# apache/paimon

Measured on AMD Instinct MI355X. Metric: merged rows/sec, higher is better.
Workload: dtype int64; 1 GPU; merge-on-read: 8 sorted runs x 10000000 rows, int64 PK + 8 int32, parquet NONE, Deduplicate, drop-delete (BASELINE.json configs[1]); n_runs=8, rows_per_run=10000000, compression=NONE, seed=42, parallelism=bucket-parallel dp1, no collectives

## Files before the change

### include/paimon_hip.h

```cpp
#ifndef PAIMON_HIP_H
#define PAIMON_HIP_H

#include <stdint.h>

#ifdef __cplusplus
extern "C" {
#endif

typedef struct pmh_session_t pmh_session_t;
typedef struct pmh_plan_t pmh_plan_t;

enum pmh_dtype {
    PMH_DT_INT8 = 1,
    PMH_DT_INT16 = 2,
    PMH_DT_INT32 = 3,
    PMH_DT_INT64 = 4,
    PMH_DT_FLOAT32 = 5,
    PMH_DT_FLOAT64 = 6,
    PMH_DT_STRING = 7,
    PMH_DT_BOOL = 8,
};

enum pmh_logical {
    PMH_LT_NONE = 0,
// ... 92 lines not shown
                              int scale, int64_t n_values, int out_esize,
                              int mode, int64_t src_shift, void *out,
                              int64_t out_cap);

int64_t pmh_debug_bits(const void *stream, int64_t len, int64_t n_values,
                       int bit_order, int format, int out_esize, int mode,
                       int64_t src_shift, int64_t out_shift, void *out,
                       int64_t out_cap);

int64_t pmh_debug_orc_timestamp(const void *data, int64_t data_len,
                                const void *secondary, int64_t secondary_len,
                                int64_t n_values, int unit, int mode,
                                void *out, int64_t out_cap);

int64_t pmh_debug_parse_dv(const char *path, int64_t offset, int64_t length,
                           int64_t *out, int64_t cap);

int pmh_debug_lookup_probe(int n_levels, const int64_t *const *level_keys,
                           const int64_t *level_rows, const int64_t *queries,
                           int64_t n_queries, int32_t *out_level,
                           int64_t *out_row);

int pmh_debug_changelog_decide(int64_t n_groups, const int32_t *nlive,
                               const int32_t *n_top,
                               const uint8_t *merged_is_add, int pending,
                               int32_t *out_n, int8_t *out_kinds,
                               uint8_t *out_after_is_merged,
                               uint8_t *out_pending);

int pmh_debug_partition(int k, const void *const *keys, const int64_t *lens,
                        int key_width, int64_t tile_rows, int mode,
                        int32_t *cuts_out);

int pmh_debug_json_i64(const char *text, int64_t *out);

int pmh_debug_interval_partition(int n, const int64_t *min_keys,
                                 const int64_t *max_keys,
                                 int32_t *out_section, int32_t *out_run);

#ifdef __cplusplus
}
#endif
#endif
```

### paimon_amd/csrc/kernels.h

```cpp
#pragma once

#include <hip/hip_runtime.h>

#include <cstdint>

#include "bits_core.h"
#include "orc_decimal_core.h"
#include "orc_timestamp_core.h"
#include "stream_core.h"

namespace pmh {

constexpr int PMH_MAX_RUNS = 32;
constexpr int PMH_ROW_BITS = 27;
constexpr uint32_t PMH_ROW_MASK = ((uint32_t)1 << PMH_ROW_BITS) - 1;
constexpr int PMH_TILE_THREADS = 512;
constexpr int64_t PMH_TILE_ROWS = 3584;
constexpr int PMH_COARSE_G = 16;
constexpr int64_t PMH_DEAD = INT64_MIN;
constexpr int PMH_TILE_MAX = PMH_TILE_ROWS + PMH_MAX_RUNS;
constexpr int PMH_TILE_ITER =
    (PMH_TILE_MAX + PMH_TILE_THREADS - 1) / PMH_TILE_THREADS;

struct DevPage {
// ... 121 lines not shown

hipError_t pmh_launch_scan_tiles(const int32_t *tile_counts, int64_t n_tiles,
                                 int64_t *tile_offsets, int64_t *total_out,
                                 hipStream_t stream);

hipError_t pmh_launch_merge_emit(const DevCol *keys, const DevCol *seqs,
                                 const DevCol *kinds, const int64_t *lens,
                                 int k, const int32_t *cuts,
                                 int64_t tile_base, int64_t tile_limit,
                                 int64_t n_tiles,
                                 int64_t tile_rows, int flags,
                                 const uint64_t *tombs,
                                 const DevCol *cols, const uint8_t *col_dtype,
                                 const uint8_t *col_nullable, int n_cols,
                                 int key_col, int seq_col, int kind_col,
                                 const int16_t *useq_cols, int n_useq,
                                 uint64_t *status, uint64_t *ticket,
                                 int64_t *total_out, uint32_t *dense_winners,
                                 void *const *out_ptrs,
                                 uint8_t *const *out_valid,
                                 uint32_t *err_flag, hipStream_t stream);

hipError_t pmh_launch_emit_dense(const DevCol *cols,
                                 const uint8_t *col_dtype,
                                 const uint8_t *col_nullable, int n_cols,
                                 int key_col, int seq_col, int kind_col,
                                 const uint32_t *winners,
                                 int64_t t0, int64_t t1,
                                 const uint64_t *status,
                                 void *const *out_ptrs,
                                 uint8_t *const *out_valid,
                                 hipStream_t stream);

hipError_t pmh_launch_emit(const DevCol *cols, const uint8_t *col_dtype,
                           const uint8_t *col_nullable, int n_cols, int k,
                           int n_desc, int contiguous,
                           const uint32_t *winners,
                           const int32_t *tile_counts,
                           const int64_t *tile_offsets, int64_t n_tiles,
                           int64_t tile_rows, const int64_t *total_out,
                           void *const *out_ptrs, uint8_t *const *out_valid,
                           hipStream_t stream);

hipError_t pmh_launch_rle_decode(const RleChunk *chunks, int64_t n_chunks,
                                 int32_t *out, hipStream_t stream);

hipError_t pmh_launch_level_scatter(const RleChunk *chunks, int64_t n_chunks,
                                    hipStream_t stream);

hipError_t pmh_launch_emit_pu(const DevCol *cols, const uint8_t *col_dtype,
                              const uint8_t *col_nullable, int n_cols, int k,
                              int seq_col, int kind_col, int flags,
                              const uint32_t *members,
                              const uint16_t *group_start,
                              const int64_t *tile_offsets, int64_t n_tiles,
                              int64_t tile_rows, const int64_t *total_out,
                              uint64_t *const *run_masks,
                              void *const *out_ptrs,
                              uint8_t *const *out_valid, hipStream_t stream);

hipError_t pmh_launch_pack_valid(const DevCol *cols, int n_cols, int64_t rows,
                                 uint64_t *mask, hipStream_t stream);

hipError_t pmh_launch_composite(const DevCol *keys, int nk, uint64_t shifts,
                                uint64_t bits, int64_t rows, int64_t *ckey,
                                hipStream_t stream);

enum {
    PMH_AGG_LAST_NON_NULL = 0,
// ... 39 lines not shown
```

### paimon_amd/csrc/kernels.hip

```cpp

#include <hip/hip_runtime.h>

#include <cstdint>
#include <cstdlib>
#include <type_traits>

#include "changelog_core.h"
#include "kernels.h"
#include "lookup_core.h"
#include "partition_core.h"
#include "zstd_core.h"

#define DEV __device__ __forceinline__

namespace pmh {


template <typename T>
DEV T col_load(const DevCol &c, int64_t row) {
    if (c.n_pages == 1)
        return *reinterpret_cast<const T *>(c.addr0 + (uint64_t)row * sizeof(T));
    int lo = 0, hi = c.n_pages - 1;
    while (lo < hi) {
        int mid = (lo + hi + 1) >> 1;
        if (c.pages[mid].start_row <= row) lo = mid;
        else hi = mid - 1;
    }
    const DevPage &pg = c.pages[lo];
    return *reinterpret_cast<const T *>(pg.addr + (uint64_t)(row - pg.start_row) * sizeof(T));
}

DEV uint64_t ukey(int64_t k) { return (uint64_t)k ^ 0x8000000000000000ull; }

DEV int64_t key_at(uint64_t addr, int64_t idx, int es) {
    return es == 8 ? *reinterpret_cast<const int64_t *>(addr + idx * 8)
                   : (int64_t)*reinterpret_cast<const int32_t *>(addr +
                                                                 idx * 4);
}


// ... 1991 lines not shown
            } else {
                wa[x] = wa[0];
            }
        }
        uint32_t packed[R];
#pragma unroll
        for (int x = 0; x < R; x++) packed[x] = gload<uint32_t>(wa[x]);
        int dl[R];
        uint32_t row[R];
#pragma unroll
        for (int x = 0; x < R; x++) {
            dl[x] = (int)(packed[x] >> PMH_ROW_BITS) * n_cols;
            row[x] = packed[x] & PMH_ROW_MASK;
        }
        auto lists = [&](auto full) {
            constexpr bool FULL = decltype(full)::value;
            const uint32_t utid = (uint32_t)tid;
            emit_list<int32_t, int8_t, G4, R, FULL>(
                s_addr, s_valid, s_out, s_ov, 0, e1, dl, row, base, utid, nr);
            emit_list<int32_t, int16_t, G4, R, FULL>(
                s_addr, s_valid, s_out, s_ov, e1, e2, dl, row, base, utid, nr);
            emit_list<int32_t, int32_t, G4, R, FULL>(
                s_addr, s_valid, s_out, s_ov, e2, e4, dl, row, base, utid, nr);
            emit_list<int64_t, int64_t, G8, R, FULL>(
                s_addr, s_valid, s_out, s_ov, e4, e8, dl, row, base, utid, nr);
        };
        if (base + (int64_t)EMIT_THREADS * R <= slice_hi)
            lists(std::true_type{});
        else
            lists(std::false_type{});
    }
}

__global__ void k_composite(const DevCol *keys, int nk, uint64_t shifts,
                            uint64_t bits, int64_t rows, int64_t *ckey) {
    const int64_t stride = (int64_t)gridDim.x * blockDim.x;
    for (int64_t i = (int64_t)blockIdx.x * blockDim.x + threadIdx.x; i < rows;
         i += stride) {
        uint64_t u = 0;
        for (int j = 0; j < nk; j++) {
            const DevCol &dc = keys[j];
            int64_t v = dc.esize == 8 ? col_load<int64_t>(dc, i)
                                      : (int64_t)col_load<int32_t>(dc, i);
            const int w = (int)((bits >> (8 * j)) & 0xff);
            const int sh = (int)((shifts >> (8 * j)) & 0xff);
            uint64_t b = ((uint64_t)v + (1ull << (w - 1))) &
                         (w >= 64 ? ~0ull : ((1ull << w) - 1));
            u |= b << sh;
        }
        ckey[i] = (int64_t)(u ^ 0x8000000000000000ull);
    }
}

__global__ void k_pack_valid(const DevCol *cols, int n_cols, int64_t rows,
                             uint64_t *mask) {
    const int64_t stride = (int64_t)gridDim.x * blockDim.x;
    for (int64_t i = (int64_t)blockIdx.x * blockDim.x + threadIdx.x; i < rows;
         i += stride) {
        uint64_t m = 0;
        for (int c = 0; c < n_cols; c++) {
            const DevCol &dc = cols[c];
            uint64_t v =
                dc.valid0 ? (uint64_t)((const uint8_t *)dc.valid0)[i] : 1u;
            m |= (v & 1) << c;
        }
        mask[i] = m;
// ... 2294 lines not shown
    };
    if (fr)
        launch(k_merge_emit<true>);
    else
        launch(k_merge_emit<false>);
    return hipGetLastError();
}

hipError_t pmh_launch_emit_dense(const DevCol *cols,
                                 const uint8_t *col_dtype,
                                 const uint8_t *col_nullable, int n_cols,
                                 int key_col, int seq_col, int kind_col,
                                 const uint32_t *winners,
                                 int64_t t0, int64_t t1,
                                 const uint64_t *status,
                                 void *const *out_ptrs,
                                 uint8_t *const *out_valid,
                                 hipStream_t stream) {
    hipLaunchKernelGGL(k_emit_dense, dim3(emit_grid()), dim3(256), 0, stream, cols,
                       col_dtype, col_nullable, n_cols, key_col, seq_col,
                       kind_col, winners, t0, t1, status, out_ptrs,
                       out_valid);
    return hipGetLastError();
}

hipError_t pmh_launch_scan_tiles(const int32_t *tile_counts, int64_t n_tiles,
                                 int64_t *tile_offsets, int64_t *total_out,
                                 hipStream_t stream) {
    hipLaunchKernelGGL(k_scan_tiles, dim3(1), dim3(PMH_TILE_THREADS), 0,
                       stream, tile_counts, n_tiles, tile_offsets, total_out);
    return hipGetLastError();
}

hipError_t pmh_launch_emit(const DevCol *cols, const uint8_t *col_dtype,
                           const uint8_t *col_nullable, int n_cols, int k,
                           int n_desc, int contiguous,
                           const uint32_t *winners,
                           const int32_t *tile_counts,
                           const int64_t *tile_offsets, int64_t n_tiles,
                           int64_t tile_rows, const int64_t *total_out,
                           void *const *out_ptrs, uint8_t *const *out_valid,
                           hipStream_t stream) {
    auto env_int = [](const char *name, int dflt) {
        const char *e = getenv(name);
        return e ? atoi(e) : dflt;
    };
    const int r_rows = env_int("PMH_EMIT_R", 4);
    const int g_cols = env_int("PMH_EMIT_G", 8);
    int n_emit = env_int("PMH_EMIT_COLS", n_cols);
    if (n_emit < 0 || n_emit > n_cols) n_emit = n_cols;
    const int grid = emit_grid();
    const int64_t lds = emit_contig_lds(n_desc, n_cols);
    const bool contig = contiguous && n_desc >= 1 && n_cols <= 256 &&
                        lds <= EMIT_LDS_MAX &&
                        env_int("PMH_EMIT_LEGACY", 0) == 0;
    if (contig) {
        auto launch = [&](auto kern) {
            hipLaunchKernelGGL(kern, dim3(grid), dim3(EMIT_THREADS), (size_t)lds,
                               stream, cols, col_dtype, col_nullable, n_cols,
                               n_emit, n_desc, winners, tile_offsets, n_tiles,
                               tile_rows, total_out, out_ptrs, out_valid);
        };
        if (r_rows == 2) {
            if (g_cols == 2) launch(k_emit_contig<2, 2, 1>);
            else if (g_cols == 4) launch(k_emit_contig<2, 4, 2>);
            else launch(k_emit_contig<2, 8, 4>);
        } else {
            if (g_cols == 2) launch(k_emit_contig<4, 2, 1>);
            else if (g_cols == 4) launch(k_emit_contig<4, 4, 2>);
            else if (g_cols == 16) launch(k_emit_contig<4, 16, 8>);
            else launch(k_emit_contig<4, 8, 4>);
        }
        return hipGetLastError();
    }
    auto launch = [&](auto kern) {
        hipLaunchKernelGGL(kern, dim3(grid), dim3(256), 0, stream, cols,
                           col_dtype, col_nullable, n_cols, n_emit, k,
                           winners, tile_counts, tile_offsets, n_tiles,
                           tile_rows, total_out, out_ptrs, out_valid);
    };
    if (r_rows == 6)
        launch(k_emit<6>);
    else if (r_rows == 8)
        launch(k_emit<8>);
    else
        launch(k_emit<4>);
    return hipGetLastError();
}
// ... 210 lines not shown
```

### paimon_amd/csrc/plan.cpp

```cpp

#include <hip/hip_runtime.h>

#include <algorithm>
#include <chrono>
#include <cstring>
#include <fstream>
#include <memory>
#include <queue>
#include <string>
#include <unordered_map>
#include <vector>

#include "../../include/paimon_hip.h"
#include "changelog_core.h"
#include "codec.h"
#include "zstd_core.h"
#include <map>
#include "common.h"
#include "json.h"
#include "kernels.h"
#include "lookup_core.h"
#include "orc_meta.h"
#include "parquet_meta.h"
#include "parquet_write.h"
// ... 3536 lines not shown
        const char *dwhat = "decode";
        hipError_t de = launch_section_decode(p, sec, st, &dwhat);
        if (de != hipSuccess) return fail(dwhat, de);
    }
    if (p->composite_key) {
        for (int r = 0; r < k; r++) {
            if (sec.runs[r].length <= 0) continue;
            hipError_t ce = pmh_launch_composite(
                sec.all_cols + (size_t)r * n_cols, p->n_key_cols,
                p->key_shifts, p->key_bits, sec.runs[r].length, sec.ckeys[r],
                st);
            if (ce != hipSuccess) return fail("composite", ce);
        }
    }
    if (sec.row_masks_dev) {
        for (int r = 0; r < k; r++) {
            if (sec.runs[r].length <= 0) continue;
            hipError_t pe = pmh_launch_pack_valid(
                sec.all_cols + (size_t)r * n_cols, n_cols,
                sec.runs[r].length, sec.row_masks[r], st);
            if (pe != hipSuccess) return fail("pack_valid", pe);
        }
    }
    (void)hipEventRecord(ev[1], st);
    if (p->filters_dev && k == 1 && !sec.hier && sec.runs[0].tomb &&
        sec.runs[0].length > 0) {
        hipError_t fe = pmh_launch_filter(
            sec.all_cols, n_cols, p->filters_dev, (int)p->filters.size(),
            sec.runs[0].length, sec.runs[0].tomb, st);
        if (fe != hipSuccess) return fail("filter", fe);
    }
    int64_t n_tiles_eff = sec.n_tiles;
    int64_t rows_eff = sec.total_rows;
    if (sec.hier) {
        const int nb = (int)sec.blo.size();
        k = nb;
        const int bflags = p->first_row ? 8 : 0;
        for (int b = 0; b < nb; b++) {
            int lo = sec.blo[b];
            int kb = sec.bhi[b] - lo;
            int64_t btiles = sec.bntiles[b];
            hipError_t hb = pmh_launch_partition(
                sec.rkeys + lo, sec.rlens + lo, kb, PMH_TILE_ROWS,
                btiles + 1, sec.brows[b], sec.cuts, st);
            if (hb != hipSuccess) return fail("hier partition", hb);
            hb = pmh_launch_merge_tiles(
                sec.rkeys + lo, sec.rseqs + lo, sec.rkinds + lo,
                sec.rlens + lo, kb, sec.cuts, btiles, PMH_TILE_ROWS, bflags,
                sec.rtombs ? sec.rtombs + lo : nullptr, sec.winners,
                sec.tile_counts, sec.group_start, sec.err_dev, nullptr, 0,
                nullptr, nullptr, nullptr, nullptr, st);
            if (hb != hipSuccess) return fail("hier merge", hb);
            hb = pmh_launch_scan_tiles(sec.tile_counts, btiles,
                                       sec.tile_offsets, sec.lens_dev + b,
                                       st);
            if (hb != hipSuccess) return fail("hier scan", hb);
            hb = pmh_launch_emit(sec.rall + (size_t)lo * n_cols,
                                 p->hier_dtype_dev, p->col_nullable_dev,
                                 n_cols, kb, kb, sec.cols_contig,
                                 sec.winners, sec.tile_counts,
                                 sec.tile_offsets, btiles, PMH_TILE_ROWS,
                                 sec.lens_dev + b, sec.bout_ptrs[b],
                                 sec.bout_valid[b], st);
            if (hb != hipSuccess) return fail("hier emit", hb);
        }
        std::vector<int64_t> vl(nb);
        if (hipMemcpy(vl.data(), sec.lens_dev, nb * 8,
                      hipMemcpyDeviceToHost) != hipSuccess)
            return fail("hier lens D2H", hipErrorUnknown);
        rows_eff = 0;
        for (int b = 0; b < nb; b++) rows_eff += vl[b];
        n_tiles_eff = (rows_eff + PMH_TILE_ROWS - 1) / PMH_TILE_ROWS;
        if (n_tiles_eff == 0) n_tiles_eff = 1;
    }
    hipError_t e = pmh_launch_partition(sec.key_cols, sec.lens_dev, k,
                                        PMH_TILE_ROWS, n_tiles_eff + 1,
                                        rows_eff, sec.cuts, st);
    if (e != hipSuccess) return fail("partition", e);
    (void)hipEventRecord(ev[2], st);
    int flags = (p->drop_delete ? 1 : 0) | (p->ignore_delete ? 2 : 0) |
                (p->pu ? 4 : 0) | (p->first_row ? 8 : 0) |
                (p->rrod ? 16 : 0) | (p->seqg ? 32 : 0) |
                (p->agg_retract ? 64 : 0);
    if (const char *ab = getenv("PMH_ABLATE"))
        flags |= (atoi(ab) & 0xf) << 8;
    if (const char *ab = getenv("PMH_FABL"))
        flags |= (atoi(ab) & 0x3) << 12;
    if (const char *fs = getenv("PMH_FSTAGE"))
        flags |= (atoi(fs) & 1) << 14;
    if (p->fused) {
        e = hipMemsetAsync(sec.status, 0, n_tiles_eff * 8, st);
        if (e != hipSuccess) return fail("status memset", e);
// ... 86 lines not shown
                               sec.run_levels, p->max_level, sec.cl_entries,
                               sec.cl_counts, sec.probe_words, sec.probe_off,
                               st);
    if (e != hipSuccess) return fail("merge_tiles", e);
    (void)hipEventRecord(ev[3], st);
    e = pmh_launch_scan_tiles(sec.tile_counts, n_tiles_eff, sec.tile_offsets,
                              sec.total_dev, st);
    if (e != hipSuccess) return fail("scan_tiles", e);
    (void)hipEventRecord(ev[4], st);
    if (p->agg) {
        e = pmh_launch_emit_agg(
            sec.all_cols, p->col_dtype_dev, p->col_nullable_dev,
            p->col_agg_dev, n_cols, k, p->n_key_cols, p->n_key_cols + 1,
            flags, sec.winners, sec.group_start, sec.tile_offsets,
            n_tiles_eff, PMH_TILE_ROWS, sec.total_dev, sec.row_masks_dev,
            p->out_ptrs_dev, p->out_valid_dev, st);
    } else if (p->pu && p->seqg) {
        e = pmh_launch_emit_pu_sg(
            sec.all_cols, p->col_dtype_dev, p->col_nullable_dev, n_cols, k,
            p->n_key_cols, p->n_key_cols + 1, flags, p->col_group_dev,
            p->sg_fields_dev, p->sg_nseq_dev, p->n_seq_groups, sec.winners,
            sec.group_start, sec.tile_offsets, n_tiles_eff, PMH_TILE_ROWS,
            sec.total_dev, sec.row_masks_dev, p->out_ptrs_dev,
            p->out_valid_dev, st);
    } else if (p->pu) {
        e = pmh_launch_emit_pu(
            sec.all_cols, p->col_dtype_dev, p->col_nullable_dev, n_cols, k,
            p->n_key_cols, p->n_key_cols + 1, flags, sec.winners,
            sec.group_start, sec.tile_offsets, n_tiles_eff, PMH_TILE_ROWS,
            sec.total_dev, sec.row_masks_dev, p->out_ptrs_dev,
            p->out_valid_dev, st);
    } else {
        e = pmh_launch_emit(sec.all_cols, p->col_dtype_dev,
                            p->col_nullable_dev, n_cols, k,
                            sec.hier ? k : k + sec.n_lookup,
                            sec.hier || sec.cols_contig, sec.winners,
                            sec.tile_counts, sec.tile_offsets, n_tiles_eff,
                            PMH_TILE_ROWS, sec.total_dev, p->out_ptrs_dev,
                            p->out_valid_dev, st);
    }
    if (e != hipSuccess) return fail("emit", e);
    if (p->cl_fold) {
        e = pmh_launch_cl_finalize_out(
            sec.all_cols, p->col_dtype_dev, p->col_nullable_dev, n_cols,
            p->n_key_cols + 2, k, sec.cl_entries, sec.cl_rows, sec.cl_counts,
            sec.tile_offsets, n_tiles_eff, PMH_TILE_ROWS, p->out_ptrs_dev,
            p->out_valid_dev, st);
        if (e != hipSuccess) return fail("cl_finalize_out", e);
        e = pmh_launch_scan_tiles(sec.cl_counts, n_tiles_eff, sec.cl_offsets,
                                  sec.cl_total_dev, st);
        if (e != hipSuccess) return fail("cl_scan", e);
        e = pmh_launch_cl_emit_out(
            sec.all_cols, p->col_dtype_dev, p->col_nullable_dev, n_cols, k,
            p->n_key_cols + 1, sec.cl_rows, sec.cl_counts, sec.cl_offsets,
            sec.tile_offsets, n_tiles_eff, PMH_TILE_ROWS, p->out_ptrs_dev,
            p->out_valid_dev, p->out_ptrs2_dev, p->out_valid2_dev, st);
        if (e != hipSuccess) return fail("cl_emit_out", e);
    } else if (p->changelog) {
        e = pmh_launch_cl_finalize(sec.all_cols, p->col_dtype_dev, n_cols,
                                   p->n_key_cols + 2, k, sec.cl_entries,
                                   sec.cl_rows, sec.cl_counts, n_tiles_eff,
                                   PMH_TILE_ROWS, st);
        if (e != hipSuccess) return fail("cl_finalize", e);
        e = pmh_launch_scan_tiles(sec.cl_counts, n_tiles_eff, sec.cl_offsets,
                                  sec.cl_total_dev, st);
        if (e != hipSuccess) return fail("cl_scan", e);
        e = pmh_launch_cl_emit(sec.all_cols, p->col_dtype_dev,
                               p->col_nullable_dev, n_cols,
                               p->n_key_cols + 1, sec.cl_rows, sec.cl_counts,
// ... 986 lines not shown
    }
    return 0;
}

int pmh_debug_changelog_decide(int64_t n_groups, const int32_t *nlive,
                               const int32_t *n_top,
                               const uint8_t *merged_is_add, int pending,
                               int32_t *out_n, int8_t *out_kinds,
                               uint8_t *out_after_is_merged,
                               uint8_t *out_pending) {
    if (n_groups < 0 ||
        (n_groups > 0 && (!nlive || !n_top || !merged_is_add || !out_n ||
                          !out_kinds))) {
        set_error("pmh_debug_changelog_decide: bad arguments");
        return -1;
    }
    for (int64_t g = 0; g < n_groups; g++) {
        if (nlive[g] < 1 || n_top[g] < 0 || n_top[g] > nlive[g]) {
            set_error("pmh_debug_changelog_decide: group %lld is malformed "
                      "(nlive >= 1, 0 <= n_top <= nlive)", (long long)g);
            return -1;
        }
        const ClcDecision d = clc_decide(nlive[g], n_top[g],
                                         merged_is_add[g] != 0, pending != 0);
        out_n[g] = d.n;
        out_kinds[2 * g] = (int8_t)(d.n >= 1 ? d.kind0 : -1);
        out_kinds[2 * g + 1] = (int8_t)(d.n == 2 ? d.kind1 : -1);
        if (out_after_is_merged) out_after_is_merged[g] = d.after_is_merged;
        if (out_pending) out_pending[g] = d.pending;
    }
    return 0;
}

int pmh_debug_partition(int k, const void *const *keys, const int64_t *lens,
                        int key_width, int64_t tile_rows, int mode,
                        int32_t *cuts_out) {
    if (k < 1 || k > PMH_MAX_RUNS || !keys || !lens || !cuts_out ||
        (key_width != 4 && key_width != 8) || tile_rows < 1 ||
        (mode != 0 && mode != 1)) {
        set_error("pmh_debug_partition: bad arguments (1..%d runs, key_width "
                  "4|8, tile_rows >= 1, mode 0|1)", PMH_MAX_RUNS);
        return -1;
    }
    int64_t total = 0;
    for (int r = 0; r < k; r++) {
        if (lens[r] < 0 || lens[r] >= ((int64_t)1 << PMH_ROW_BITS) ||
            (lens[r] > 0 && !keys[r])) {
            set_error("pmh_debug_partition: run %d is malformed", r);
            return -1;
        }
        total += lens[r];
    }
    const int64_t n_bounds = (total + tile_rows - 1) / tile_rows + 1;
    if (mode == 0) {
        const int64_t G = k <= 8 ? (n_bounds > PMH_COARSE_G + 1 ? PMH_COARSE_G
                                                                 : 1)
                                 : (n_bounds > 1 ? n_bounds - 1 : 1);
        static_assert(PPC_MAX_RUNS == PMH_MAX_RUNS, "widest instantiation");
        ppc_host_partition(k, keys, lens, key_width, tile_rows, n_bounds,
                           total, G, cuts_out);
        return 0;
    }
    constexpr int GUARD = 64;
    const size_t n_cuts = (size_t)n_bounds * k;
    std::vector<void *> bufs;
    auto dalloc = [&](size_t n) -> void * {
// ... 102 lines not shown
```

### paimon_amd/reader.py

```python

import ctypes
import json
import os

import numpy as np

_HERE = os.path.dirname(os.path.abspath(__file__))
LIB_PATH = os.path.join(_HERE, "libpaimon_hip.so")

_DT_NP = {1: np.int8, 2: np.int16, 3: np.int32, 4: np.int64,
          5: np.float32, 6: np.float64,
          7: np.int32,
          8: np.bool_}

(LT_NONE, LT_DATE, LT_TIME_MILLIS, LT_TIMESTAMP_MILLIS, LT_TIMESTAMP_MICROS,
 LT_TIMESTAMP_LTZ_MILLIS, LT_TIMESTAMP_LTZ_MICROS) = range(7)


class _Col(ctypes.Structure):
    _fields_ = [("name", ctypes.c_char_p), ("dtype", ctypes.c_int32),
                ("data", ctypes.c_void_p), ("valid", ctypes.c_void_p),
                ("dict_data", ctypes.c_void_p),
                ("dict_offsets", ctypes.POINTER(ctypes.c_int32)),
                ("dict_len", ctypes.c_int32),
# ... 399 lines not shown
    return out_level, out_row


PARTITION_HOST = 0
PARTITION_DEVICE = 1


def debug_partition(runs, tile_rows, mode=PARTITION_HOST):
    lib = load_lib()
    dt = np.dtype(runs[0].dtype)
    if dt not in (np.dtype(np.int64), np.dtype(np.int32)):
        raise ValueError("keys must be int64 or int32")
    ks = [np.ascontiguousarray(a, dtype=dt) for a in runs]
    k = len(ks)
    total = sum(len(a) for a in ks)
    n_bounds = (total + tile_rows - 1) // tile_rows + 1
    ptrs = (ctypes.c_void_p * k)(
        *[a.ctypes.data if len(a) else None for a in ks])
    lens = (ctypes.c_int64 * k)(*[len(a) for a in ks])
    cuts = np.empty((n_bounds, k), dtype=np.int32)
    lib.pmh_debug_partition.restype = ctypes.c_int
    lib.pmh_debug_partition.argtypes = [
        ctypes.c_int, ctypes.POINTER(ctypes.c_void_p),
        ctypes.POINTER(ctypes.c_int64), ctypes.c_int, ctypes.c_int64,
        ctypes.c_int, ctypes.POINTER(ctypes.c_int32)]
    rc = lib.pmh_debug_partition(
        k, ptrs, lens, dt.itemsize, tile_rows, mode,
        cuts.ctypes.data_as(ctypes.POINTER(ctypes.c_int32)))
    if rc != 0:
        raise RuntimeError(last_error())
    return cuts


class Session:
    def __init__(self, device=0):
        self.lib = load_lib()
        self.h = self.lib.pmh_open_session(device)
        if not self.h:
            raise RuntimeError(f"pmh_open_session: {last_error()}")
        self.device = device

    def close(self):
        if self.h:
            self.lib.pmh_close_session(self.h)
            self.h = None

    def __enter__(self):
        return self

    def __exit__(self, *a):
        self.close()


class MergeReadPlan:

    def __init__(self, session: Session, files, key_cols, value_cols,
                 merge_engine="deduplicate", drop_delete=True,
                 ignore_delete=False, output="host", aggregations=None,
                 remove_record_on_delete=False, sequence_groups=None,
                 ignore_retract=None, sequence_fields=None,
                 changelog_producer=None, changelog_row_dedup=False,
                 max_level=None, sort_engine="loser-tree", filters=None,
                 lookup_files=None):
        self.lib = session.lib
        desc = {
            "key_cols": key_cols,
# ... 134 lines not shown
```

Measured before the change: 20.87 billion rows/s.

## Add streamed LDS-staged emit kernel that gathers tile source rows then permutes winners

Adds a new emit path for contiguous, non-nullable inputs. Each tile's source rows are read coalesced from the sorted runs and grouped by column width into LDS. Winners are then gathered from LDS via slot indices computed from the tile cuts. The loads for the next column group or next tile are issued before the current permute, overlapping global reads with LDS work. This replaces scattered random global gathers with sequential loads, at the cost of reading loser rows too, added LDS pressure and barriers, and a more complex persistent-grid schedule.

```diff
diff --git a/include/paimon_hip.h b/include/paimon_hip.h
--- a/include/paimon_hip.h
+++ b/include/paimon_hip.h
@@ -148,6 +148,8 @@
                         int key_width, int64_t tile_rows, int mode,
                         int32_t *cuts_out);
 
+int pmh_debug_last_emit_kernel(void);
+
 int pmh_debug_json_i64(const char *text, int64_t *out);
 
 int pmh_debug_interval_partition(int n, const int64_t *min_keys,
diff --git a/paimon_amd/csrc/emit_stream_core.h b/paimon_amd/csrc/emit_stream_core.h
--- /dev/null
+++ b/paimon_amd/csrc/emit_stream_core.h
@@ -0,0 +1,101 @@
+#ifndef PMH_EMIT_STREAM_CORE_H
+#define PMH_EMIT_STREAM_CORE_H
+
+#include <stdint.h>
+
+#if defined(__HIPCC__)
+#define ESC_HD __host__ __device__ __forceinline__
+#else
+#define ESC_HD inline
+#endif
+#if defined(__clang__)
+#define ESC_UNROLL _Pragma("unroll")
+#else
+#define ESC_UNROLL
+#endif
+
+template <int KM>
+struct EscTile {
+    int32_t a[KM];
+    int32_t len[KM];
+    int32_t segoff[KM];
+    int32_t mtotal;
+    int32_t mreal;
+};
+
+template <int KM>
+ESC_HD void esc_tile_setup(const int32_t *c0, const int32_t *c1,
+                           const int64_t *lens, int k, EscTile<KM> &t) {
+    int32_t so = 0, mr = 0;
+    ESC_UNROLL
+    for (int r = 0; r < KM; r++) {
+        const int rr = r < k ? r : 0;
+        const int32_t ar = c0[rr], br = c1[rr];
+        const int32_t ln = (int32_t)lens[rr];
+        t.a[r] = ar;
+        t.len[r] = r < k ? (br - ar) + (br < ln ? 1 : 0) : 0;
+        t.segoff[r] = so;
+        so += t.len[r];
+        mr += r < k ? br - ar : 0;
+    }
+    t.mtotal = so;
+    t.mreal = mr;
+}
+
+template <int KM>
+ESC_HD void esc_slot_source(const EscTile<KM> &t, int k, int32_t e, int *run,
+                            uint32_t *row) {
+    int rn = 0;
+    int32_t rowd = 0;
+    ESC_UNROLL
+    for (int r = 0; r < KM; r++) {
+        const bool in = r < k && e >= t.segoff[r];
+        rn = in ? r : rn;
+        rowd = in ? t.a[r] - t.segoff[r] : rowd;
+    }
+    *run = rn;
+    *row = (uint32_t)(e + rowd);
+}
+
+template <int KM>
+ESC_HD int32_t esc_winner_slot(const EscTile<KM> &t, uint32_t run,
+                               uint32_t row) {
+    int32_t off = 0;
+    ESC_UNROLL
+    for (int r = 0; r < KM; r++)
+        off = run == (uint32_t)r ? t.segoff[r] - t.a[r] : off;
+    return (int32_t)row + off;
+}
+
+ESC_HD int esc_stored_width(int cls) { return cls == 8 ? 8 : 4; }
+
+ESC_HD int64_t esc_col_bytes(int cls, int has_valid, int tile_max) {
+    return (int64_t)tile_max * (esc_stored_width(cls) + (has_valid ? 1 : 0));
+}
+
+ESC_HD int esc_plan_groups(const uint8_t *cls, const uint8_t *valid, int n,
+                           int tile_max, int64_t budget, int max4, int max8,
+                           uint16_t *bound) {
+    int g = 0;
+    bound[0] = 0;
+    int i = 0;
+    while (i < n) {
+        const int c = cls[i];
+        const int cap = esc_stored_width(c) == 8 ? max8 : max4;
+        int64_t used = 0;
+        int j = i;
+        while (j < n && cls[j] == c && j - i < cap) {
+            const int64_t b =
+                esc_col_bytes(c, valid ? valid[j] : 0, tile_max);
+            if (used + b > budget) break;
+            used += b;
+            j++;
+        }
+        if (j == i) return -1;
+        bound[++g] = (uint16_t)j;
+        i = j;
+    }
+    return g;
+}
+
+#endif
diff --git a/paimon_amd/csrc/emit_stream_hostcheck.cpp b/paimon_amd/csrc/emit_stream_hostcheck.cpp
--- /dev/null
+++ b/paimon_amd/csrc/emit_stream_hostcheck.cpp
@@ -0,0 +1,237 @@
+#include "emit_stream_core.h"
+
+#include <cstdio>
+#include <cstdlib>
+#include <random>
+#include <vector>
+
+static int failures = 0;
+
+#define CHECK(cond)                                                        \
+    do {                                                                   \
+        if (!(cond)) {                                                     \
+            fprintf(stderr, "%s:%d: CHECK failed: %s\n", __FILE__,         \
+                    __LINE__, #cond);                                      \
+            failures++;                                                    \
+        }                                                                  \
+    } while (0)
+
+static const int MAX_RUNS = 32;
+static const int64_t TILE_ROWS = 3584;
+static const int TILE_MAX = (int)TILE_ROWS + MAX_RUNS;
+
+static std::vector<int32_t> gen_cuts(const std::vector<int64_t> &lens,
+                                     std::mt19937_64 &rng, int skew) {
+    const int k = (int)lens.size();
+    int64_t total = 0;
+    for (int64_t l : lens) total += l;
+    const int64_t n_tiles = total ? (total + TILE_ROWS - 1) / TILE_ROWS : 1;
+    std::vector<int32_t> cuts((size_t)(n_tiles + 1) * k, 0);
+    std::vector<int64_t> at(k, 0);
+    for (int64_t b = 1; b <= n_tiles; b++) {
+        int64_t want = b * TILE_ROWS < total ? TILE_ROWS
+                                             : total - (b - 1) * TILE_ROWS;
+        while (want > 0) {
+            int r = (int)(rng() % k);
+            if (skew && (rng() % (unsigned)(skew + 1)))
+                r = (int)(rng() % (unsigned)((k + 1) / 2));
+            if (at[r] >= lens[r]) {
+                r = -1;
+                for (int q = 0; q < k; q++)
+                    if (at[q] < lens[q]) r = q;
+                if (r < 0) break;
+            }
+            int64_t take = 1 + (int64_t)(rng() % 97);
+            if (take > want) take = want;
+            if (take > lens[r] - at[r]) take = lens[r] - at[r];
+            at[r] += take;
+            want -= take;
+        }
+        for (int r = 0; r < k; r++) cuts[(size_t)b * k + r] = (int32_t)at[r];
+    }
+    return cuts;
+}
+
+template <int KM>
+static void check_tiles(const std::vector<int64_t> &lens,
+                        const std::vector<int32_t> &cuts) {
+    const int k = (int)lens.size();
+    const int64_t n_tiles = (int64_t)cuts.size() / k - 1;
+    CHECK(k <= KM);
+    std::vector<int64_t> hl(lens);
+    for (int64_t t = 0; t < n_tiles; t++) {
+        std::vector<int32_t> c0(cuts.begin() + t * k,
+                                cuts.begin() + (t + 1) * k);
+        std::vector<int32_t> c1(cuts.begin() + (t + 1) * k,
+                                cuts.begin() + (t + 2) * k);
+        EscTile<KM> ts;
+        esc_tile_setup<KM>(c0.data(), c1.data(), hl.data(), k, ts);
+        const int32_t M = ts.mtotal;
+        CHECK(M >= 0 && M <= TILE_MAX);
+        int64_t real = 0, ext = 0;
+        for (int r = 0; r < k; r++) {
+            real += c1[r] - c0[r];
+            ext += c1[r] < lens[r] ? 1 : 0;
+        }
+        CHECK(ts.mreal == real);
+        CHECK(M == real + ext);
+        CHECK(real <= TILE_ROWS);
+        for (int32_t e = 0; e < M; e++) {
+            int run = -1;
+            uint32_t row = 0;
+            esc_slot_source<KM>(ts, k, e, &run, &row);
+            CHECK(run >= 0 && run < k);
+            if (run < 0 || run >= k) continue;
+            CHECK((int64_t)row >= c0[run] && (int64_t)row <= c1[run]);
+            CHECK((int64_t)row < lens[run]);
+            CHECK(esc_winner_slot<KM>(ts, (uint32_t)run, row) == e);
+        }
+        std::vector<uint8_t> hit((size_t)M, 0);
+        int64_t named = 0;
+        for (int r = 0; r < k; r++) {
+            for (int64_t row = c0[r]; row <= c1[r] && row < lens[r]; row++) {
+                const int32_t s =
+                    esc_winner_slot<KM>(ts, (uint32_t)r, (uint32_t)row);
+                CHECK(s >= 0 && s < M);
+                if (s < 0 || s >= M) continue;
+                CHECK(!hit[(size_t)s]);
+                hit[(size_t)s] = 1;
+                named++;
+            }
+        }
+        CHECK(named == M);
+    }
+}
+
+static void check_runs(const std::vector<int64_t> &lens,
+                       const std::vector<int32_t> &cuts) {
+    const int k = (int)lens.size();
+    if (k <= 4) check_tiles<4>(lens, cuts);
+    if (k <= 8) check_tiles<8>(lens, cuts);
+    if (k <= 16) check_tiles<16>(lens, cuts);
+    check_tiles<32>(lens, cuts);
+}
+
+static void tiles() {
+    std::mt19937_64 rng(20240611);
+    const int ks[] = {1, 2, 3, 8, 32};
+    for (int k : ks) {
+        for (int rep = 0; rep < 6; rep++) {
+            std::vector<int64_t> lens(k);
+            for (int r = 0; r < k; r++)
+                lens[r] = (int64_t)(rng() % (rep < 2 ? 300 : 9000));
+            if (rep == 3) lens[0] = 1;
+            if (rep == 4) lens[k - 1] = 0;
+            if (rep == 5 && k > 1) lens[1] = 20000;
+            check_runs(lens, gen_cuts(lens, rng, rep >= 3 ? 3 : 0));
+        }
+    }
+    {
+        const int64_t totals[] = {TILE_ROWS, TILE_ROWS + 1, 2 * TILE_ROWS, 100};
+        for (int64_t tot : totals) {
+            std::vector<int64_t> one{tot};
+            check_runs(one, gen_cuts(one, rng, 0));
+            std::vector<int64_t> three{1, tot / 2, tot - tot / 2 - 1};
+            check_runs(three, gen_cuts(three, rng, 2));
+        }
+    }
+    {
+        const int k = MAX_RUNS;
+        const int64_t per = TILE_ROWS / k;
+        std::vector<int64_t> lens(k, 2 * per);
+        std::vector<int32_t> cuts((size_t)3 * k, 0);
+        for (int r = 0; r < k; r++) {
+            cuts[(size_t)k + r] = (int32_t)per;
+            cuts[(size_t)2 * k + r] = (int32_t)(2 * per);
+        }
+        check_tiles<32>(lens, cuts);
+        EscTile<32> ts;
+        esc_tile_setup<32>(cuts.data(), cuts.data() + k, lens.data(), k, ts);
+        CHECK(ts.mtotal == TILE_MAX);
+        esc_tile_setup<32>(cuts.data() + k, cuts.data() + 2 * k, lens.data(),
+                           k, ts);
+        CHECK(ts.mtotal == TILE_ROWS);
+    }
+    {
+        std::vector<int64_t> lens{10, 5000};
+        std::vector<int32_t> cuts{0, 0, 10, 3574, 10, 5000};
+        check_runs(lens, cuts);
+    }
+}
+
+static void check_plan(const std::vector<uint8_t> &cls,
+                       const std::vector<uint8_t> *valid, int64_t budget,
+                       int max4, int max8) {
+    const int n = (int)cls.size();
+    std::vector<uint16_t> bound((size_t)n + 1, 0xffff);
+    const int g = esc_plan_groups(cls.data(), valid ? valid->data() : nullptr,
+                                  n, TILE_MAX, budget, max4, max8,
+                                  bound.data());
+    bool fits = true;
+    for (int i = 0; i < n; i++)
+        fits = fits &&
+               esc_col_bytes(cls[i], valid ? (*valid)[i] : 0, TILE_MAX) <=
+                   budget;
+    if (!fits) {
+        CHECK(g == -1);
+        return;
+    }
+    CHECK(g >= (n ? 1 : 0) && g <= n);
+    if (g < 0) return;
+    CHECK(bound[0] == 0 && bound[(size_t)g] == n);
+    for (int i = 0; i < g; i++) {
+        const int lo = bound[(size_t)i], hi = bound[(size_t)i + 1];
+        CHECK(lo < hi && hi <= n);
+        if (!(lo < hi && hi <= n)) return;
+        int64_t bytes = 0;
+        for (int c = lo; c < hi; c++) {
+            CHECK(cls[c] == cls[lo]);
+            bytes += esc_col_bytes(cls[c], valid ? (*valid)[c] : 0, TILE_MAX);
+        }
+        CHECK(bytes <= budget);
+        CHECK(hi - lo <= (esc_stored_width(cls[lo]) == 8 ? max8 : max4));
+    }
+}
+
+static void plans() {
+    std::mt19937_64 rng(7);
+    const int ns[] = {1, 12, 13, 256};
+    const int64_t budgets[] = {1000,       (int64_t)TILE_MAX * 4,
+                               (int64_t)TILE_MAX * 8, 60 * 1024,
+                               (int64_t)TILE_MAX * 32 + 5};
+    const int caps[][2] = {{2, 1}, {4, 2}, {8, 4}};
+    for (int n : ns) {
+        for (int rep = 0; rep < 4; rep++) {
+            std::vector<uint8_t> cls((size_t)n), valid((size_t)n);
+            const uint8_t widths[] = {1, 2, 4, 8};
+            for (int i = 0; i < n; i++) {
+                cls[(size_t)i] =
+                    rep == 0 ? 4 : widths[(size_t)i * 4 / (size_t)n];
+                if (rep == 2) cls[(size_t)i] = i < n / 3 ? 4 : 8;
+                valid[(size_t)i] = (uint8_t)(rng() & 1);
+            }
+            for (int64_t b : budgets)
+                for (const auto &cp : caps) {
+                    check_plan(cls, nullptr, b, cp[0], cp[1]);
+                    check_plan(cls, &valid, b, cp[0], cp[1]);
+                }
+        }
+    }
+    std::vector<uint8_t> cls{1, 4, 4, 4, 4, 4, 4, 4, 4, 8, 8, 8};
+    uint16_t bound[13];
+    CHECK(esc_plan_groups(cls.data(), nullptr, 12, TILE_MAX, 60 * 1024, 4, 2,
+                          bound) == 5);
+    CHECK(bound[1] == 1 && bound[2] == 5 && bound[3] == 9 && bound[4] == 11 &&
+          bound[5] == 12);
+}
+
+int main() {
+    tiles();
+    plans();
+    if (failures) {
+        fprintf(stderr, "emit_stream_hostcheck: %d failure(s)\n", failures);
+        return 1;
+    }
+    printf("emit_stream_hostcheck OK\n");
+    return 0;
+}
diff --git a/paimon_amd/csrc/kernels.h b/paimon_amd/csrc/kernels.h
--- a/paimon_amd/csrc/kernels.h
+++ b/paimon_amd/csrc/kernels.h
@@ -177,9 +177,18 @@
                                  uint8_t *const *out_valid,
                                  hipStream_t stream);
 
+enum {
+    PMH_EMIT_NONE = 0,
+    PMH_EMIT_PAGED = 1,
+    PMH_EMIT_CONTIG = 2,
+    PMH_EMIT_STREAM = 3,
+};
+int pmh_last_emit_kernel();
+
 hipError_t pmh_launch_emit(const DevCol *cols, const uint8_t *col_dtype,
-                           const uint8_t *col_nullable, int n_cols, int k,
-                           int n_desc, int contiguous,
+                           const uint8_t *col_nullable, int any_nullable,
+                           int n_cols, int k, int n_desc, int contiguous,
+                           const int32_t *cuts, const int64_t *lens,
                            const uint32_t *winners,
                            const int32_t *tile_counts,
                            const int64_t *tile_offsets, int64_t n_tiles,
diff --git a/paimon_amd/csrc/kernels.hip b/paimon_amd/csrc/kernels.hip
--- a/paimon_amd/csrc/kernels.hip
+++ b/paimon_amd/csrc/kernels.hip
@@ -6,6 +6,7 @@
 #include <type_traits>
 
 #include "changelog_core.h"
+#include "emit_stream_core.h"
 #include "kernels.h"
 #include "lookup_core.h"
 #include "partition_core.h"
@@ -2063,6 +2064,248 @@
     }
 }
 
+constexpr int EMS_THREADS = PMH_TILE_THREADS;
+constexpr int EMS_ITER = PMH_TILE_ITER;
+constexpr int64_t EMS_LDS_DEFAULT = 60 * 1024;
+
+__host__ __device__ static inline int64_t emit_stream_tables(int64_t k,
+                                                             int64_t n_cols) {
+    const int64_t b = 8 * k * n_cols + 8 * n_cols + 32 +
+                      2 * (n_cols + 1) + 3 * n_cols;
+    return (b + 15) & ~(int64_t)15;
+}
+
+template <typename T>
+DEV T ems_keep(T x) {
+    asm volatile("" : "+v"(x));
+    return x;
+}
+
+template <int W, int GU>
+DEV void ems_load(const uint64_t *s_addr, int p, int n, int n_cols,
+                  const uint32_t (&src)[EMS_ITER],
+                  uint32_t (&v)[GU][EMS_ITER]) {
+#pragma unroll
+    for (int g = 0; g < GU * 4 / W; g++) {
+        if (g >= n) break;
+#pragma unroll
+        for (int s = 0; s < EMS_ITER; s++) {
+            const uint32_t sr = ems_keep(src[s]);
+            const uint64_t a =
+                s_addr[(sr >> PMH_ROW_BITS) * (uint32_t)n_cols + p + g] +
+                (uint64_t)((sr & PMH_ROW_MASK) * (uint32_t)W);
+            if constexpr (W == 8) {
+                const uint64_t x = gload<uint64_t>(a);
+                v[2 * g][s] = (uint32_t)x;
+                v[2 * g + 1][s] = (uint32_t)(x >> 32);
+            } else {
+                v[g][s] = gload<uint32_t>(a);
+            }
+        }
+        __builtin_amdgcn_sched_barrier(0);
+    }
+}
+
+template <int W, int GU>
+DEV void ems_fill(uint8_t *buf, int n, int32_t m, int tid,
+                  const uint32_t (&v)[GU][EMS_ITER]) {
+#pragma unroll
+    for (int g = 0; g < GU * 4 / W; g++) {
+        if (g >= n) break;
+        const int32_t t = ems_keep(tid);
+#pragma unroll
+        for (int s = 0; s < EMS_ITER; s++) {
+            const int32_t e = t + s * EMS_THREADS;
+            if (e >= m) continue;
+            uint8_t *d = buf + ((size_t)g * PMH_TILE_MAX + e) * W;
+            if constexpr (W == 8)
+                *reinterpret_cast<uint64_t *>(d) =
+                    ((uint64_t)v[2 * g + 1][s] << 32) | v[2 * g][s];
+            else
+                *reinterpret_cast<uint32_t *>(d) = v[g][s];
+        }
+    }
+}
+
+template <typename L, typename S>
+DEV void ems_permute(const uint8_t *buf, const uint64_t *s_out, int p, int n,
+                     int64_t toff, int32_t count, int tid,
+                     const uint32_t (&wslot)[EMS_ITER / 2]) {
+    for (int g = 0; g < n; g++) {
+        const uint64_t ob =
+            uniform64(s_out[p + g] + (uint64_t)toff * sizeof(S));
+        const uint8_t *cb = buf + (size_t)g * PMH_TILE_MAX * sizeof(L);
+        const int32_t t = ems_keep(tid);
+#pragma unroll
+        for (int s = 0; s < EMS_ITER; s++) {
+            const int32_t j = t + s * EMS_THREADS;
+            if (j >= count) continue;
+            const L x = *reinterpret_cast<const L *>(
+                cb + (size_t)((ems_keep(wslot[s / 2]) >> (16 * (s & 1))) &
+                              0xffffu) *
+                         sizeof(L));
+            const uint64_t oa =
+                ob + (uint64_t)((uint32_t)t * (uint32_t)sizeof(S)) +
+                (uint64_t)(s * EMS_THREADS * (int)sizeof(S));
+            gstore<S>(oa, (S)x);
+        }
+    }
+}
+
+template <int KM, int GU>
+__attribute__((amdgpu_waves_per_eu(4))) __launch_bounds__(EMS_THREADS, 2)
+__global__
+void k_emit_stream(const DevCol *cols ,
+                   const uint8_t *col_dtype, int n_cols, int n_emit, int k,
+                   const int32_t *__restrict__ cuts,
+                   const int64_t *__restrict__ lens,
+                   const uint32_t *__restrict__ winners,
+                   const int32_t *__restrict__ tile_counts,
+                   const int64_t *__restrict__ tile_offsets, int64_t n_tiles,
+                   int64_t tile_rows, void *const *out_ptrs,
+                   int lds_budget) {
+    extern __shared__ uint64_t ems_smem[];
+    const int n_ent = k * n_cols;
+    uint64_t *s_addr = ems_smem;
+    uint64_t *s_out = s_addr + n_ent;
+    int *s_cnt = (int *)(s_out + n_cols);
+    uint16_t *s_bound = (uint16_t *)(s_cnt + 8);
+    uint8_t *s_pos = (uint8_t *)(s_bound + n_cols + 1);
+    uint8_t *s_cls = s_pos + n_cols;
+    uint8_t *s_clsp = s_cls + n_cols;
+    uint8_t *buf =
+        (uint8_t *)ems_smem + emit_stream_tables(k, n_cols);
+
+    const int tid = threadIdx.x;
+    auto dt_class = [](int dt) {
+        return dt == 1 ? 1
+               : dt == 2 ? 2
+               : (dt == 3 || dt == 5 || dt == 7) ? 4
+               : (dt == 4 || dt == 6) ? 8
+                                      : 0;
+    };
+    for (int c = tid; c < n_cols; c += EMS_THREADS)
+        s_cls[c] = c < n_emit ? dt_class(col_dtype[c]) : 0;
+    __syncthreads();
+    for (int c = tid; c < n_cols; c += EMS_THREADS) {
+        const int cls = s_cls[c];
+        int n_of[4] = {0, 0, 0, 0};
+        int before = 0;
+        for (int j = 0; j < n_cols; j++) {
+            const int cj = s_cls[j];
+#pragma unroll
+            for (int w = 0; w < 4; w++) n_of[w] += cj == (1 << w);
+            before += (j < c && cj == cls);
+        }
+        if (c == 0) {
+#pragma unroll
+            for (int w = 0; w < 4; w++) s_cnt[w] = n_of[w];
+        }
+        if (cls) {
+            int p = before;
+#pragma unroll
+            for (int w = 0; w < 3; w++) p += (1 << w) < cls ? n_of[w] : 0;
+            s_pos[c] = (uint8_t)p;
+            s_clsp[p] = (uint8_t)cls;
+            s_out[p] = (uint64_t)out_ptrs[c];
+        }
+    }
+    __syncthreads();
+    for (int e = tid; e < n_ent; e += EMS_THREADS) {
+        const int r = e / n_cols, c = e - r * n_cols;
+        if (!s_cls[c]) continue;
+        s_addr[r * n_cols + s_pos[c]] = cols[e].addr0;
+    }
+    if (tid == 0)
+        s_cnt[4] = esc_plan_groups(
+            s_clsp, nullptr, s_cnt[0] + s_cnt[1] + s_cnt[2] + s_cnt[3],
+            PMH_TILE_MAX, lds_budget, GU, GU / 2, s_bound);
+    __syncthreads();
+    const int ng = s_cnt[4];
+    int64_t tile = blockIdx.x;
+    if (ng <= 0 || tile >= n_tiles) return;
+
+    const int64_t wstride = tile_rows + PMH_MAX_RUNS;
+    EscTile<KM> ts;
+    uint32_t src[EMS_ITER];
+    uint32_t wraw[EMS_ITER], v[GU][EMS_ITER];
+    uint32_t wslot[EMS_ITER / 2];
+    int32_t count_n;
+    int64_t toff_n;
+    auto setup = [&](int64_t t) {
+        asm volatile("" : "+s"(t));
+        esc_tile_setup<KM>(cuts + t * k, cuts + (t + 1) * k, lens, k, ts);
+        count_n = tile_counts[t];
+        toff_n = tile_offsets[t];
+        const int32_t last = ts.mtotal > 0 ? ts.mtotal - 1 : 0;
+        const int32_t tk = ems_keep(tid);
+#pragma unroll
+        for (int s = 0; s < EMS_ITER; s++) {
+            const int32_t x = tk + s * EMS_THREADS;
+            int run;
+            uint32_t row;
+            esc_slot_source<KM>(ts, k, x < last ? x : last, &run, &row);
+            src[s] = ((uint32_t)run << PMH_ROW_BITS) | row;
+        }
+        const uint64_t wb = (uint64_t)(winners + t * wstride);
+        const uint32_t wlast = (uint32_t)wstride - 1;
+#pragma unroll
+        for (int s = 0; s < EMS_ITER; s++) {
+            const uint32_t j = (uint32_t)(tk + s * EMS_THREADS);
+            wraw[s] = gload<uint32_t>(wb + (j < wlast ? j : wlast) * 4u);
+        }
+    };
+    auto issue = [&](int gi) {
+        if (ts.mtotal <= 0) return;
+        const int p = s_bound[gi], n = s_bound[gi + 1] - p;
+        if (s_clsp[p] == 8) ems_load<8, GU>(s_addr, p, n, n_cols, src, v);
+        else ems_load<4, GU>(s_addr, p, n, n_cols, src, v);
+    };
+    setup(tile);
+    issue(0);
+    for (;;) {
+        const int32_t count = count_n;
+        const int64_t toff = toff_n;
+#pragma unroll
+        for (int s = 0; s < EMS_ITER; s += 2) {
+            const uint32_t lo = (uint32_t)esc_winner_slot<KM>(
+                ts, wraw[s] >> PMH_ROW_BITS, wraw[s] & PMH_ROW_MASK);
+            const uint32_t hi = (uint32_t)esc_winner_slot<KM>(
+                ts, wraw[s + 1] >> PMH_ROW_BITS, wraw[s + 1] & PMH_ROW_MASK);
+            wslot[s / 2] = (lo & 0xffffu) | (hi << 16);
+        }
+        const int64_t next = tile + gridDim.x;
+        for (int gi = 0; gi < ng; gi++) {
+            const int p = s_bound[gi], n = s_bound[gi + 1] - p;
+            const int cls = s_clsp[p];
+            if (cls == 8) ems_fill<8, GU>(buf, n, ts.mtotal, tid, v);
+            else ems_fill<4, GU>(buf, n, ts.mtotal, tid, v);
+            if (gi + 1 < ng) {
+                issue(gi + 1);
+            } else if (next < n_tiles) {
+                setup(next);
+                issue(0);
+            }
+            __syncthreads();
+            if (cls == 1)
+                ems_permute<int32_t, int8_t>(buf, s_out, p, n, toff,
+                                                 count, tid, wslot);
+            else if (cls == 2)
+                ems_permute<int32_t, int16_t>(buf, s_out, p, n, toff,
+                                                  count, tid, wslot);
+            else if (cls == 4)
+                ems_permute<int32_t, int32_t>(buf, s_out, p, n, toff,
+                                                  count, tid, wslot);
+            else
+                ems_permute<int64_t, int64_t>(buf, s_out, p, n, toff,
+                                                  count, tid, wslot);
+            __syncthreads();
+        }
+        if (next >= n_tiles) break;
+        tile = next;
+    }
+}
+
 __global__ void k_composite(const DevCol *keys, int nk, uint64_t shifts,
                             uint64_t bits, int64_t rows, int64_t *ckey) {
     const int64_t stride = (int64_t)gridDim.x * blockDim.x;
@@ -4423,9 +4666,13 @@
     return hipGetLastError();
 }
 
+static int g_last_emit_kernel = PMH_EMIT_NONE;
+int pmh_last_emit_kernel() { return g_last_emit_kernel; }
+
 hipError_t pmh_launch_emit(const DevCol *cols, const uint8_t *col_dtype,
-                           const uint8_t *col_nullable, int n_cols, int k,
-                           int n_desc, int contiguous,
+                           const uint8_t *col_nullable, int any_nullable,
+                           int n_cols, int k, int n_desc, int contiguous,
+                           const int32_t *cuts, const int64_t *lens,
                            const uint32_t *winners,
                            const int32_t *tile_counts,
                            const int64_t *tile_offsets, int64_t n_tiles,
@@ -4445,6 +4692,43 @@
     const bool contig = contiguous && n_desc >= 1 && n_cols <= 256 &&
                         lds <= EMIT_LDS_MAX &&
                         env_int("PMH_EMIT_LEGACY", 0) == 0;
+    const int64_t tables = emit_stream_tables(k, n_cols);
+    const bool streamed = contig && n_desc == k && !any_nullable &&
+                          tables <= EMIT_LDS_MAX && cuts && lens &&
+                          tile_rows == PMH_TILE_ROWS &&
+                          env_int("PMH_EMIT_STREAM", 1) != 0;
+    if (streamed) {
+        int64_t budget = env_int("PMH_EMIT_STREAM_LDS", (int)EMS_LDS_DEFAULT);
+        const int64_t col8 = (int64_t)PMH_TILE_MAX * 8;
+        if (budget < col8) budget = col8;
+        if (budget > EMS_LDS_DEFAULT) budget = EMS_LDS_DEFAULT;
+        if (budget > 64 * 1024 - tables) budget = 64 * 1024 - tables;
+        const int gu = budget >= 2 * col8 ? 4 : 2;
+        int64_t max_blocks = 4096;
+        if (const char *e = getenv("PMH_EMIT_STREAM_BLOCKS")) {
+            const long long v = atoll(e);
+            if (v >= 1 && v <= 65535) max_blocks = v;
+        }
+        const int blocks = n_tiles < max_blocks ? (int)n_tiles : (int)max_blocks;
+        const size_t bytes = (size_t)(tables + budget);
+        auto launch = [&](auto kern) {
+            hipLaunchKernelGGL(kern, dim3(blocks), dim3(EMS_THREADS), bytes,
+                               stream, cols, col_dtype, n_cols, n_emit, k,
+                               cuts, lens, winners, tile_counts, tile_offsets,
+                               n_tiles, tile_rows, out_ptrs, (int)budget);
+        };
+        auto launch_g = [&](auto km) {
+            constexpr int KM = decltype(km)::value;
+            if (gu == 2) launch(k_emit_stream<KM, 2>);
+            else launch(k_emit_stream<KM, 4>);
+        };
+        if (k <= 8) launch_g(std::integral_constant<int, 8>{});
+        else if (k <= 16) launch_g(std::integral_constant<int, 16>{});
+        else launch_g(std::integral_constant<int, PMH_MAX_RUNS>{});
+        g_last_emit_kernel = PMH_EMIT_STREAM;
+        return hipGetLastError();
+    }
+    g_last_emit_kernel = contig ? PMH_EMIT_CONTIG : PMH_EMIT_PAGED;
     if (contig) {
         auto launch = [&](auto kern) {
             hipLaunchKernelGGL(kern, dim3(grid), dim3(EMIT_THREADS), (size_t)lds,
diff --git a/paimon_amd/csrc/plan.cpp b/paimon_amd/csrc/plan.cpp
--- a/paimon_amd/csrc/plan.cpp
+++ b/paimon_amd/csrc/plan.cpp
@@ -3592,6 +3592,8 @@
     }
     int64_t n_tiles_eff = sec.n_tiles;
     int64_t rows_eff = sec.total_rows;
+    int any_nullable = 0;
+    for (bool nb : p->col_nullable) any_nullable |= nb ? 1 : 0;
     if (sec.hier) {
         const int nb = (int)sec.blo.size();
         k = nb;
@@ -3617,7 +3619,8 @@
             if (hb != hipSuccess) return fail("hier scan", hb);
             hb = pmh_launch_emit(sec.rall + (size_t)lo * n_cols,
                                  p->hier_dtype_dev, p->col_nullable_dev,
-                                 n_cols, kb, kb, sec.cols_contig,
+                                 any_nullable, n_cols, kb, kb,
+                                 sec.cols_contig, sec.cuts, sec.rlens + lo,
                                  sec.winners, sec.tile_counts,
                                  sec.tile_offsets, btiles, PMH_TILE_ROWS,
                                  sec.lens_dev + b, sec.bout_ptrs[b],
@@ -3770,9 +3773,10 @@
             p->out_valid_dev, st);
     } else {
         e = pmh_launch_emit(sec.all_cols, p->col_dtype_dev,
-                            p->col_nullable_dev, n_cols, k,
+                            p->col_nullable_dev, any_nullable, n_cols, k,
                             sec.hier ? k : k + sec.n_lookup,
-                            sec.hier || sec.cols_contig, sec.winners,
+                            sec.hier || sec.cols_contig, sec.cuts,
+                            sec.lens_dev, sec.winners,
                             sec.tile_counts, sec.tile_offsets, n_tiles_eff,
                             PMH_TILE_ROWS, sec.total_dev, p->out_ptrs_dev,
                             p->out_valid_dev, st);
@@ -4825,6 +4829,8 @@
     return 0;
 }
 
+int pmh_debug_last_emit_kernel(void) { return pmh_last_emit_kernel(); }
+
 int pmh_debug_partition(int k, const void *const *keys, const int64_t *lens,
                         int key_width, int64_t tile_rows, int mode,
                         int32_t *cuts_out) {
diff --git a/paimon_amd/reader.py b/paimon_amd/reader.py
--- a/paimon_amd/reader.py
+++ b/paimon_amd/reader.py
@@ -455,6 +455,16 @@
     return cuts
 
 
+EMIT_NONE, EMIT_PAGED, EMIT_CONTIG, EMIT_STREAM = 0, 1, 2, 3
+
+
+def debug_last_emit_kernel():
+    lib = load_lib()
+    lib.pmh_debug_last_emit_kernel.restype = ctypes.c_int
+    lib.pmh_debug_last_emit_kernel.argtypes = []
+    return int(lib.pmh_debug_last_emit_kernel())
+
+
 class Session:
     def __init__(self, device=0):
         self.lib = load_lib()
```

Measured after the change: 22.60 billion rows/s (median of 6 runs). 1.08x the previous value.
